# OSU-Nowlab/MPI4DL

Hardware: NVIDIA H100
Metric: images/sec (device-timed, max over ranks) AmoebaNet-D 8192^2 hot path (spatial-stage conv/pool fwd+bwd) (higher is better)
Workload: dtype bf16

## Files before the change

mpi4dl_b200/build.py:

```python
import os
import subprocess
import sys

HERE = os.path.dirname(os.path.abspath(__file__))
CSRC = os.path.join(HERE, "csrc")
LIB = os.path.join(HERE, "libspconv.so")
SOURCES = ["api.cu", "conv_direct.cu", "pool.cu", "halo.cu", "gemm_tc.cu", "conv_tap.cu", "wgrad_tap.cu", "bnrelu.cu",
           "halo_grad.cu", "gemm_tf32.cu", "conv_tap_tf32.cu", "conv_tap_s2_tf32.cu",
           "gemm_px.cu"]
NVCC_FLAGS = [
    "-O3", "-std=c++17", "-gencode", "arch=compute_90a,code=sm_90a", "-lineinfo",
    "-Xcompiler", "-fPIC", "--expt-relaxed-constexpr",
]


def _stale(target, deps):
    if not os.path.exists(target):
        return True
    t = os.path.getmtime(target)
    return any(os.path.getmtime(d) > t for d in deps)


def build_lib(force=False, verbose=False):
    nvcc = os.environ.get("NVCC", "/usr/local/cuda/bin/nvcc")
    hdrs = [os.path.join(CSRC, f) for f in os.listdir(CSRC) if f.endswith((".cuh", ".h"))]
    hdrs.append(os.path.join(HERE, "..", "include", "spconv.h"))
    objs = []
    procs = []
    for s in SOURCES:
        src = os.path.join(CSRC, s)
        obj = os.path.join(CSRC, s.replace(".cu", ".o"))
        objs.append(obj)
        if force or _stale(obj, [src] + hdrs):
            cmd = [nvcc] + NVCC_FLAGS + (["-Xptxas", "-v"] if verbose else []) + ["-c", src, "-o", obj]
            procs.append((s, subprocess.Popen(cmd, stdout=subprocess.PIPE, stderr=subprocess.STDOUT, text=True)))
    for s, p in procs:
        out, _ = p.communicate()
        if p.returncode != 0:
            sys.stderr.write(out)
            raise RuntimeError("nvcc failed on %s" % s)
        if verbose:
            sys.stderr.write(out)
    if force or procs or _stale(LIB, objs):
        cmd = [nvcc, "-shared", "-o", LIB] + objs + ["-gencode", "arch=compute_90a,code=sm_90a"]
        subprocess.check_call(cmd)
    return LIB


if __name__ == "__main__":
    print(build_lib(force="--force" in sys.argv, verbose="-v" in sys.argv))
```

mpi4dl_b200/csrc/gemm_tc.cu:

```cuda
#include <stdlib.h>

#include "common.cuh"
#include "tc_common.cuh"

namespace spc {

using namespace tc;

bool tap_v2_supported(int M, int Cin, int R, int S, int H, int W, int N, int stride);
int run_conv_tap_v2(const __nv_bfloat16* wp, int Mpad, int Cpad, const __nv_bfloat16* x, const __nv_bfloat16* bias,
                    __nv_bfloat16* y, int M, int Cin, int R, int S, int ph, int H, int W, int N, cudaStream_t st);

bool wgrad_tap_supported(int K, int C, int R, int S, int H, int W, int stride);
int run_wgrad_tap(const __nv_bfloat16* x, const __nv_bfloat16* dy, float* dw, int K, int C, int N, int H, int W, int R, int S,
                  cudaStream_t st);

int run_pw_px(int NT, const CUtensorMap& tw, const CUtensorMap& tx, const CUtensorMap& ty, int M, int Cin, int N, int P,
              int x5, int y5, const __nv_bfloat16* bias, int sms, cudaStream_t st);

namespace {

constexpr int TC_THREADS = 384;
constexpr int BK = 64;
constexpr int A_BLK_BYTES = 128 * BK * 2;
constexpr int B_BLK_BYTES = BK * 64 * 2;

typedef CUresult (*EncodeTiledFn)(CUtensorMap*, CUtensorMapDataType, cuuint32_t, void*, const cuuint64_t*,
                                  const cuuint64_t*, const cuuint32_t*, const cuuint32_t*, CUtensorMapInterleave,
                                  CUtensorMapSwizzle, CUtensorMapL2promotion, CUtensorMapFloatOOBfill);
EncodeTiledFn get_encode() {
  static EncodeTiledFn fn = nullptr;
  if (!fn) {
    void* p = nullptr;
    cudaDriverEntryPointQueryResult q;
    if (cudaGetDriverEntryPoint("cuTensorMapEncodeTiled", &p, cudaEnableDefault, &q) == cudaSuccess &&
        q == cudaDriverEntryPointSuccess)
      fn = reinterpret_cast<EncodeTiledFn>(p);
  }
  return fn;
}

int make_tmap_sw(CUtensorMap* m, const void* base, int rank, const uint64_t* dims, const uint64_t* strides_bytes,
                 const uint32_t* box, CUtensorMapSwizzle swz) {
  EncodeTiledFn enc = get_encode();
  if (!enc) {
    set_error("cuTensorMapEncodeTiled entry point not available");
    return SPC_ECUDA;
  }
  static thread_local bool ctx_bound = false;
  if (!ctx_bound) {
    if (cudaFree(nullptr) != cudaSuccess) {
      set_error("wgmma conv: no CUDA context on this thread");
      return SPC_ECUDA;
    }
    ctx_bound = true;
  }
  cuuint64_t gd[5], gs[5];
  cuuint32_t bx[5], es[5];
  for (int i = 0; i < rank; ++i) {
    gd[i] = dims[i];
    bx[i] = box[i];
    es[i] = 1;
    if (i > 0) gs[i - 1] = strides_bytes[i];
  }
  CUresult r = enc(m, CU_TENSOR_MAP_DATA_TYPE_BFLOAT16, (cuuint32_t)rank, const_cast<void*>(base), gd, gs, bx, es,
                   CU_TENSOR_MAP_INTERLEAVE_NONE, swz, CU_TENSOR_MAP_L2_PROMOTION_L2_256B,
                   CU_TENSOR_MAP_FLOAT_OOB_FILL_NONE);
  if (r != CUDA_SUCCESS) {
    set_error("cuTensorMapEncodeTiled failed (%d) rank=%d dims=[%llu,%llu,%llu] strides=[%llu,%llu]", (int)r, rank,
              (unsigned long long)dims[0], (unsigned long long)(rank > 1 ? dims[1] : 0),
              (unsigned long long)(rank > 2 ? dims[2] : 0), (unsigned long long)(rank > 1 ? strides_bytes[1] : 0),
              (unsigned long long)(rank > 2 ? strides_bytes[2] : 0));
    return SPC_ECUDA;
  }
  return SPC_OK;
}

int make_tmap(CUtensorMap* m, const void* base, int rank, const uint64_t* dims, const uint64_t* strides_bytes,
              const uint32_t* box) {
  return make_tmap_sw(m, base, rank, dims, strides_bytes, box, CU_TENSOR_MAP_SWIZZLE_128B);
}

__global__ void repack_weights_kernel(const __nv_bfloat16* __restrict__ w, __nv_bfloat16* __restrict__ wp, int M,
                                      int Cc, int Mpad, int Cpad, int taps, long long sm, long long sc, int flip) {
  const int total = taps * Mpad * Cpad;
  for (int i = blockIdx.x * blockDim.x + threadIdx.x; i < total; i += gridDim.x * blockDim.x) {
    const int c = i % Cpad;
    const int m = (i / Cpad) % Mpad;
    const int tap = i / (Cpad * Mpad);
    __nv_bfloat16 v = __float2bfloat16(0.f);
    if (m < M && c < Cc) v = w[(size_t)m * sm + (size_t)c * sc + (flip ? taps - 1 - tap : tap)];
    wp[i] = v;
  }
}
// ... 215 lines not shown
  }
  return sms;
}

constexpr int SMEM_LIMIT = 222 * 1024;
constexpr int SMEM_AUX = 1024  + 512 ;

template <int MB>
int launch_pw(const CUtensorMap& tw, const CUtensorMap& tx, const CUtensorMap& tx4, const CUtensorMap& ty, PwParams p,
              cudaStream_t st) {
  const int kchunks = (p.Cin + BK - 1) / BK;
  const int budget = SMEM_LIMIT - SMEM_AUX;
  const int wres_bytes = p.taps * kchunks * MB * A_BLK_BYTES;
  const int sms = sm_count();
  const int grid = p.num_tiles < sms ? p.num_tiles : sms;
  if (p.num_tiles < 16 * sms) p.tgroup = 1;
  p.wres = (wres_bytes <= 128 * 1024 && p.num_mg == 1) ? 1 : 0;
  const int stage_bytes = (p.wres ? 0 : MB * A_BLK_BYTES) + (BN / 64) * B_BLK_BYTES;
  const int rem = budget - (p.wres ? wres_bytes : 0);
  p.out_bufs = 2;
  p.stages = (rem - 2 * OUT_BUF_BYTES) / stage_bytes;
  if (p.stages < 3) { p.out_bufs = 1; p.stages = (rem - OUT_BUF_BYTES) / stage_bytes; }
  if (p.stages > MAX_STAGES) p.stages = MAX_STAGES;
  SPC_REQUIRE(p.stages >= 2, "wgmma conv: shared memory budget too small (MB=%d kchunks=%d)", MB, kchunks);
  const int smem = (p.wres ? wres_bytes : 0) + p.stages * stage_bytes + p.out_bufs * OUT_BUF_BYTES + SMEM_AUX;
  auto kern = pw_gemm_kernel<MB>;
  static bool attr_set = false;
  if (!attr_set) {
    SPC_CHECK_CUDA(cudaFuncSetAttribute(kern, cudaFuncAttributeMaxDynamicSharedMemorySize, SMEM_LIMIT));
    attr_set = true;
  }
  kern<<<grid, TC_THREADS, smem, st>>>(tw, tx, tx4, ty, p);
  count_launch();
  SPC_CHECK_CUDA(cudaGetLastError());
  return SPC_OK;
}

int make_act_tmap(CUtensorMap* m, const void* base, int P, int Cc, int N, int box_rows) {
  const uint64_t dims[3] = {(uint64_t)P, (uint64_t)Cc, (uint64_t)N};
  const uint64_t strides[3] = {0, (uint64_t)P * 2, (uint64_t)P * Cc * 2};
  const uint32_t box[3] = {64, (uint32_t)box_rows, 1};
  return make_tmap(m, base, 3, dims, strides, box);
}

int make_act_tmap5(CUtensorMap* m, const void* base, int P, int Cc, int N, int groups, int blocks) {
  const uint64_t dims[5] = {64, 8, (uint64_t)P / 64, (uint64_t)Cc / 8, (uint64_t)N};
  const uint64_t strides[5] = {0, (uint64_t)P * 2, 128, (uint64_t)P * 16, (uint64_t)P * Cc * 2};
  const uint32_t box[5] = {64, 8, (uint32_t)blocks, (uint32_t)groups, 1};
  return make_tmap(m, base, 5, dims, strides, box);
}

int launch_shift_copies(const void* x, void* xs, size_t planes, int H, int W, int S, int pw, int cs, cudaStream_t st);

struct TcConv {
  const __nv_bfloat16* w;
  long long sm, sc;
  int flip;
  int M, Cin;
  int R, S, ph, pw;
  int H, W, N;
  int stride;
  const __nv_bfloat16* prepacked;
  int px;
};

int px_tile_channels(int M) {
  const int nt = M <= 56 ? 56 : (M <= 104 ? 104 : 208);
  const int pad = round_up(M, nt);
  const int blocks = (M + 127) / 128;
  const int old_rows = (blocks >= 2 ? round_up(blocks, 2) : 1) * 128;
  return (pad < old_rows && 10 * M >= 9 * pad) ? nt : 0;
}

int run_conv_tc(const TcConv& c, const __nv_bfloat16* x, const __nv_bfloat16* bias, __nv_bfloat16* y, void* ws,
                size_t ws_bytes, cudaStream_t st) {
  const int taps = c.R * c.S;
  const int cs = c.stride;
  const int Ho = c.H / cs, Wo = c.W / cs;
  const int Pin = c.H * c.W, P = Ho * Wo;
  const int nt = (c.px && taps == 1) ? px_tile_channels(c.M) : 0;
  const bool px = nt && (long long)c.N * ((P + BN - 1) / BN) >= 2ll * sm_count();
  const int Mpad = round_up(c.M, px ? nt : 128), Cpad = round_up(c.Cin, BK);
  const bool v2 = taps > 1 && !env_get("SPC_TAP_V1") && tap_v2_supported(c.M, c.Cin, c.R, c.S, c.H, c.W, c.N, cs);
  const bool copies = (c.S > 1 || cs > 1) && taps > 1 && !v2;
  const uintptr_t ws0 = reinterpret_cast<uintptr_t>(ws);
  const uintptr_t wp_addr = (ws0 + 1023) & ~(uintptr_t)1023;
  const size_t wp_bytes = c.prepacked ? 0 : (size_t)taps * Mpad * Cpad * 2;
  const uintptr_t xs_addr = (wp_addr + wp_bytes + 1023) & ~(uintptr_t)1023;
  const size_t xs_bytes = copies ? (size_t)c.S * c.N * c.Cin * c.H * Wo * 2 : 0;
  const size_t need = (xs_addr - ws0) + xs_bytes;
  SPC_REQUIRE((ws && ws_bytes >= need) || need <= 1024, "wgmma conv: workspace too small (%zu < %zu)", ws_bytes, need);
  const __nv_bfloat16* wp = c.prepacked;
  if (!c.prepacked) {
    __nv_bfloat16* wpm = reinterpret_cast<__nv_bfloat16*>(wp_addr);
    const int total = taps * Mpad * Cpad;
    int blocks = (total + 255) / 256;
    if (blocks > 1184) blocks = 1184;
    repack_weights_kernel<<<blocks, 256, 0, st>>>(c.w, wpm, c.M, c.Cin, Mpad, Cpad, taps, c.sm, c.sc, c.flip);
    count_launch();
    SPC_CHECK_CUDA(cudaGetLastError());
    wp = wpm;
  }
  if (v2)
    return run_conv_tap_v2(wp, Mpad, Cpad, x, bias, y, c.M, c.Cin, c.R, c.S, c.ph, c.H, c.W, c.N, st);
  const __nv_bfloat16* xsrc = x;
  if (copies) {
    void* xs = reinterpret_cast<void*>(xs_addr);
    int rc0 = launch_shift_copies(x, xs, (size_t)c.N * c.Cin, c.H, c.W, c.S, c.pw, cs, st);
    if (rc0) return rc0;
    xsrc = reinterpret_cast<const __nv_bfloat16*>(xs);
  }
  CUtensorMap tw, tx, tx4, ty;
  const char* box5_env = env_get("SPC_PW_BOX5");
  const int box5 = box5_env ? atoi(box5_env) : ((size_t)P * 2 >= ((size_t)4 << 20) ? 3 : 0);
  const int x5 = (taps == 1 && cs == 1 && (box5 & 1) && P % 64 == 0 && c.Cin % 8 == 0) ? 1 : 0;
  const int y5 = (taps == 1 && (box5 & 2) && P % 64 == 0 && c.M % 8 == 0) ? 1 : 0;
  {
    const uint64_t dims[2] = {(uint64_t)Cpad, (uint64_t)taps * Mpad};
    const uint64_t strides[2] = {0, (uint64_t)Cpad * 2};
    const uint32_t box[2] = {BK, px ? (uint32_t)nt : 128u};
    int rc = make_tmap(&tw, wp, 2, dims, strides, box);
    if (rc) return rc;
  }
  int rc;
  if (px) {
    rc = x5 ? make_act_tmap5(&tx, x, Pin, c.Cin, c.N, BK / 8, BN / 64) : make_act_tmap(&tx, x, Pin, c.Cin, c.N, BK);
    if (rc) return rc;
    rc = y5 ? make_act_tmap5(&ty, y, P, c.M, c.N, nt / 8, 2) : make_act_tmap(&ty, y, P, c.M, c.N, nt);
    if (rc) return rc;
    return run_pw_px(nt, tw, tx, ty, c.M, c.Cin, c.N, P, x5, y5, bias, sm_count(), st);
  }
  if (taps > 1) {
    const uint64_t dims[4] = {(uint64_t)Wo, (uint64_t)c.H, (uint64_t)c.Cin, (uint64_t)c.N * (copies ? c.S : 1)};
    const uint64_t strides[4] = {0, (uint64_t)Wo * 2, (uint64_t)c.H * Wo * 2, (uint64_t)c.H * Wo * c.Cin * 2};
    const uint32_t box[4] = {64, 1, BK, 1};
    rc = make_tmap(&tx4, xsrc, 4, dims, strides, box);
    if (rc) return rc;
    tx = tx4;
  } else {
    rc = x5 ? make_act_tmap5(&tx, x, Pin, c.Cin, c.N, BK / 8, BN / 64) : make_act_tmap(&tx, x, Pin, c.Cin, c.N, BK);
    if (rc) return rc;
    tx4 = tx;
  }
  rc = y5 ? make_act_tmap5(&ty, y, P, c.M, c.N, 16, 2) : make_act_tmap(&ty, y, P, c.M, c.N, 128);
  if (rc) return rc;
  PwParams p{};
  p.x5 = x5; p.y5 = y5;
  p.bias = bias; p.M = c.M; p.Cin = c.Cin; p.P = P; p.N = c.N;
  p.taps = taps; p.S = c.S; p.ph = c.ph; p.pw = c.pw; p.W = Wo; p.Mpad = Mpad;
  p.shiftN = copies ? c.N : 0;
  p.rowmul = cs;
  {
    const char* e = env_get("SPC_TILE_GROUP");
    p.tgroup = e ? atoi(e) : 1;
    if (p.tgroup < 1) p.tgroup = 1;
  }
  const int MBtot = Mpad / 128;
  const int mb = MBtot >= 2 ? 2 : 1;
  p.num_mg = (MBtot + mb - 1) / mb;
  p.tiles_per_image = (P + BN - 1) / BN;
  p.num_tiles = p.tiles_per_image * c.N * p.num_mg;
  return mb == 2 ? launch_pw<2>(tw, tx, tx4, ty, p, st) : launch_pw<1>(tw, tx, tx4, ty, p, st);
}

int run_pw(const __nv_bfloat16* w, int ld, int transpose, int M, int Cin, const __nv_bfloat16* x,
           const __nv_bfloat16* bias, __nv_bfloat16* y, int N, int P, void* ws, size_t ws_bytes, cudaStream_t st,
           int px = 1) {
  TcConv c{};
  c.px = px;
  c.w = w;
  c.sm = transpose ? 1 : ld; c.sc = transpose ? ld : 1; c.flip = 0;
  c.M = M; c.Cin = Cin; c.R = 1; c.S = 1; c.ph = 0; c.pw = 0; c.H = 1; c.W = P; c.N = N; c.stride = 1;
  return run_conv_tc(c, x, bias, y, ws, ws_bytes, st);
}

constexpr int WG_ACC = 256;

struct WgParams {
  float* dw;
  int K, C, P, N;
  int nblk;
  int n_blocks;
  int MG;
  int mgroups;
  int splits;
// ... 492 lines not shown
    count_launch();
    SPC_CHECK_CUDA(cudaGetLastError());
    return SPC_OK;
  }
  if (aligned && cs == 2 && S == 3 && pw == 1 && W % 16 == 0) {
    const size_t tot = planes * H * (W / 16);
    size_t blocks = (tot + 255) / 256;
    if (blocks > 132 * 32) blocks = 132 * 32;
    shift_copies_s2k3_kernel<<<(int)blocks, 256, 0, st>>>((const __nv_bfloat16*)x, (__nv_bfloat16*)xs, planes, H, W);
    count_launch();
    SPC_CHECK_CUDA(cudaGetLastError());
    return SPC_OK;
  }
  const size_t total = planes * H * (W / cs / 8) * S;
  size_t blocks = (total + 255) / 256;
  if (blocks > 132 * 32) blocks = 132 * 32;
  shift_copies_kernel<<<(int)blocks, 256, 0, st>>>((const __nv_bfloat16*)x, (__nv_bfloat16*)xs, planes, H, W, S, pw, cs);
  count_launch();
  SPC_CHECK_CUDA(cudaGetLastError());
  return SPC_OK;
}

inline bool is_s2(const spc_conv_desc* d) { return d->stride_h == 2 && d->stride_w == 2; }
inline size_t align1k(size_t b) { return (b + 1023) & ~(size_t)1023; }

bool tap_shape_ok(const spc_conv_desc* d) {
  if (d->dtype != SPC_BF16) return false;
  if (d->R * d->S == 1 || d->R * d->S > 49) return false;
  if ((d->R & 1) == 0 || (d->S & 1) == 0) return false;
  const bool s1 = d->stride_h == 1 && d->stride_w == 1, s2 = d->stride_h == 2 && d->stride_w == 2;
  if (!s1 && !s2) return false;
  if (s2 && (d->H % 2 || d->W % 2)) return false;
  const int Wo = d->W / d->stride_w;
  if (Wo % 64 != 0) return false;
  return (long long)d->H * d->W < (1ll << 31);
}

bool pw_shape_ok(const spc_conv_desc* d) {
  if (d->dtype != SPC_BF16) return false;
  if (d->R != 1 || d->S != 1) return false;
  long long P = (long long)d->H * d->W;
  if (is_s2(d)) {
    if (d->H % 2 || d->W % 32) return false;
    P /= 4;
  } else if (d->stride_h != 1 || d->stride_w != 1) {
    return false;
  }
  if (P % 8 != 0 || P >= (1ll << 31)) return false;
  return true;
}

}

bool tc_supported(const spc_conv_desc* d, int op) {
  if (pw_shape_ok(d)) return true;
  if (tap_shape_ok(d)) {
    if (tc_workspace_bytes(d, op) > (24ull << 30)) return false;
    if (op == 1 && is_s2(d)) return d->R == 3 && d->S == 3 && 4 * d->C <= 2048;
    return true;
  }
  return false;
}

static size_t wbytes(const spc_conv_desc* d, int op) {
  const size_t taps = (size_t)d->R * d->S;
  if (op == 0) return align1k(taps * round_up(d->K, 128) * round_up(d->C, BK) * 2 + 1024);
  if (op == 1) return align1k(taps * round_up(d->C, 128) * round_up(d->K, BK) * 2 + 1024);
  return 0;
}
size_t tc_workspace_bytes(const spc_conv_desc* d, int op) {
  const size_t taps = (size_t)d->R * d->S;
  const int cs = d->stride_w;
  size_t b = wbytes(d, op) + 4096;
  if (taps == 1) {
    if (is_s2(d)) b += align1k((size_t)d->N * d->C * (d->H / 2) * (d->W / 2) * 2) + 1024;
    return b;
  }
  const size_t Ho = d->H / cs, Wo = d->W / cs;
  if (op == 1 && is_s2(d)) {
    b = align1k(4ull * round_up(4 * d->C, 128) * round_up(d->K, BK) * 2) + 4096;
    b += align1k(2ull * d->N * d->K * Ho * Wo * 2) + align1k(4ull * d->N * d->C * Ho * Wo * 2) + 4096;
    return b;
  }
  if (op != 2 && !env_get("SPC_TAP_V1") &&
      tap_v2_supported(op == 1 ? d->C : d->K, op == 1 ? d->K : d->C, d->R, d->S, d->H, d->W, d->N, cs))
    return b;
  if (op == 2 && !env_get("SPC_TAP_V1") && wgrad_tap_supported(d->K, d->C, d->R, d->S, d->H, d->W, cs))
    return b;
  if (d->S > 1 || cs > 1)
    b += align1k((size_t)d->S * d->N * (op == 1 ? d->K : d->C) * d->H * Wo * 2) + 2048;
  return b;
}

int tc_conv_fwd(const spc_conv_desc* d, const void* x, const void* w, const void* bias, void* y, void* ws,
                size_t ws_bytes, cudaStream_t st) {
  SPC_REQUIRE(ws && ws_bytes >= tc_workspace_bytes(d, 0), "wgmma conv: workspace too small");
  if (d->R * d->S > 1) {
    TcConv c{};
    c.w = reinterpret_cast<const __nv_bfloat16*>(w);
    c.sm = (long long)d->C * d->R * d->S; c.sc = (long long)d->R * d->S; c.flip = 0;
    c.M = d->K; c.Cin = d->C; c.R = d->R; c.S = d->S; c.ph = d->pad_h; c.pw = d->pad_w;
    c.H = d->H; c.W = d->W; c.N = d->N; c.stride = d->stride_h;
    return run_conv_tc(c, reinterpret_cast<const __nv_bfloat16*>(x), reinterpret_cast<const __nv_bfloat16*>(bias),
                       reinterpret_cast<__nv_bfloat16*>(y), ws, ws_bytes, st);
  }
  if (is_s2(d)) {
    void* xs = reinterpret_cast<void*>(align1k(reinterpret_cast<uintptr_t>(ws) + wbytes(d, 0)));
    int rc = launch_resample(false, x, xs, (size_t)d->N * d->C, d->H, d->W, st);
    if (rc) return rc;
    return run_pw(reinterpret_cast<const __nv_bfloat16*>(w), d->C, 0, d->K, d->C,
                  reinterpret_cast<const __nv_bfloat16*>(xs), reinterpret_cast<const __nv_bfloat16*>(bias),
                  reinterpret_cast<__nv_bfloat16*>(y), d->N, (d->H / 2) * (d->W / 2), ws, wbytes(d, 0), st);
  }
  return run_pw(reinterpret_cast<const __nv_bfloat16*>(w), d->C, 0, d->K, d->C,
                reinterpret_cast<const __nv_bfloat16*>(x), reinterpret_cast<const __nv_bfloat16*>(bias),
                reinterpret_cast<__nv_bfloat16*>(y), d->N, d->H * d->W, ws, ws_bytes, st);
}

int tc_conv_dgrad(const spc_conv_desc* d, const void* dy, const void* w, void* dx, void* ws, size_t ws_bytes,
                  cudaStream_t st) {
  SPC_REQUIRE(ws && ws_bytes >= tc_workspace_bytes(d, 1), "wgmma conv: workspace too small");
  if (d->R * d->S > 1 && is_s2(d)) {
    const int Ho = d->H / 2, Wo = d->W / 2;
    const int Mq = 4 * d->C, Mpad = round_up(Mq, 128), Kpad = round_up(d->K, BK);
    uintptr_t a = align1k(reinterpret_cast<uintptr_t>(ws));
    __nv_bfloat16* wq = reinterpret_cast<__nv_bfloat16*>(a);
    a = align1k(a + (size_t)4 * Mpad * Kpad * 2);
    __nv_bfloat16* tmp = reinterpret_cast<__nv_bfloat16*>(a);
    a = align1k(a + (size_t)4 * d->N * d->C * Ho * Wo * 2);
    {
      const int total = 4 * Mpad * Kpad;
      int blocks = (total + 255) / 256;
      if (blocks > 1184) blocks = 1184;
      repack_dgrad_s2_kernel<<<blocks, 256, 0, st>>>(reinterpret_cast<const __nv_bfloat16*>(w), wq, d->K, d->C, Mpad, Kpad);
      count_launch();
      SPC_CHECK_CUDA(cudaGetLastError());
    }
    TcConv c{};
    c.prepacked = wq;
    c.M = Mq; c.Cin = d->K; c.R = 2; c.S = 2; c.ph = 0; c.pw = 0; c.H = Ho; c.W = Wo; c.N = d->N; c.stride = 1;
    int rc = run_conv_tc(c, reinterpret_cast<const __nv_bfloat16*>(dy), nullptr, tmp, reinterpret_cast<void*>(a),
                         ws_bytes - (a - reinterpret_cast<uintptr_t>(ws)), st);
    if (rc) return rc;
    const size_t total = (size_t)d->N * d->C * 2 * Ho * (Wo / 8);
    size_t blocks = (total + 255) / 256;
    if (blocks > 132 * 32) blocks = 132 * 32;
    interleave_s2_kernel<<<(int)blocks, 256, 0, st>>>(tmp, reinterpret_cast<__nv_bfloat16*>(dx), d->N, d->C, Ho, Wo);
    count_launch();
    SPC_CHECK_CUDA(cudaGetLastError());
    return SPC_OK;
  }
  if (d->R * d->S > 1) {
    TcConv c{};
    c.w = reinterpret_cast<const __nv_bfloat16*>(w);
    c.sm = (long long)d->R * d->S; c.sc = (long long)d->C * d->R * d->S; c.flip = 1;
    c.M = d->C; c.Cin = d->K; c.R = d->R; c.S = d->S; c.ph = d->R - 1 - d->pad_h; c.pw = d->S - 1 - d->pad_w;
    c.H = d->H; c.W = d->W; c.N = d->N; c.stride = 1;
    return run_conv_tc(c, reinterpret_cast<const __nv_bfloat16*>(dy), nullptr, reinterpret_cast<__nv_bfloat16*>(dx), ws,
                       ws_bytes, st);
  }
  if (is_s2(d)) {
    void* gs = reinterpret_cast<void*>(align1k(reinterpret_cast<uintptr_t>(ws) + wbytes(d, 1)));
    int rc = run_pw(reinterpret_cast<const __nv_bfloat16*>(w), d->C, 1, d->C, d->K,
                    reinterpret_cast<const __nv_bfloat16*>(dy), nullptr, reinterpret_cast<__nv_bfloat16*>(gs), d->N,
                    (d->H / 2) * (d->W / 2), ws, wbytes(d, 1), st);
    if (rc) return rc;
    return launch_resample(true, gs, dx, (size_t)d->N * d->C, d->H, d->W, st);
  }
  return run_pw(reinterpret_cast<const __nv_bfloat16*>(w), d->C, 1, d->C, d->K,
                reinterpret_cast<const __nv_bfloat16*>(dy), nullptr, reinterpret_cast<__nv_bfloat16*>(dx), d->N,
                d->H * d->W, ws, ws_bytes, st);
}

int tc_conv_wgrad(const spc_conv_desc* d, const void* x, const void* dy, float* dw, int accumulate, void* ws,
                  size_t ws_bytes, cudaStream_t st) {
  (void)accumulate;
  const __nv_bfloat16* xb = reinterpret_cast<const __nv_bfloat16*>(x);
  const __nv_bfloat16* dyb = reinterpret_cast<const __nv_bfloat16*>(dy);
  if (d->R * d->S > 1) {
    const int cs = d->stride_h;
    if (!env_get("SPC_TAP_V1") && wgrad_tap_supported(d->K, d->C, d->R, d->S, d->H, d->W, cs))
      return run_wgrad_tap(xb, dyb, dw, d->K, d->C, d->N, d->H, d->W, d->R, d->S, st);
    const bool copies = d->S > 1 || cs > 1;
    if (copies) {
      SPC_REQUIRE(ws && ws_bytes >= tc_workspace_bytes(d, 2), "wgmma wgrad: workspace too small");
      void* xs = reinterpret_cast<void*>(align1k(reinterpret_cast<uintptr_t>(ws)));
      int rc = launch_shift_copies(x, xs, (size_t)d->N * d->C, d->H, d->W, d->S, d->pad_w, cs, st);
      if (rc) return rc;
      xb = reinterpret_cast<const __nv_bfloat16*>(xs);
    }
    return run_wgrad(xb, dyb, dw, d->K, d->C, d->N, d->H / cs, d->W / cs, d->H, d->R, d->S, d->pad_h, cs, copies, st);
  }
  if (is_s2(d)) {
    SPC_REQUIRE(ws && ws_bytes >= tc_workspace_bytes(d, 2), "wgmma wgrad: workspace too small");
    void* xs = reinterpret_cast<void*>(align1k(reinterpret_cast<uintptr_t>(ws)));
    int rc = launch_resample(false, x, xs, (size_t)d->N * d->C, d->H, d->W, st);
    if (rc) return rc;
    return run_wgrad(reinterpret_cast<const __nv_bfloat16*>(xs), dyb, dw, d->K, d->C, d->N, 1, (d->H / 2) * (d->W / 2), 1,
                     1, 1, 0, 1, false, st);
  }
  return run_wgrad(xb, dyb, dw, d->K, d->C, d->N, 1, d->H * d->W, 1, 1, 1, 0, 1, false, st);
}

size_t tc_pw_workspace_bytes(int M, int Cin) { return (size_t)round_up(M, 128) * round_up(Cin, BK) * 2 + 4096; }
int tc_pw_fwd(const void* w, int ld, int M, int Cin, const void* x, const void* bias, void* y, int P, void* ws, size_t ws_bytes,
              cudaStream_t st) {
  return run_pw(reinterpret_cast<const __nv_bfloat16*>(w), ld, 0, M, Cin, reinterpret_cast<const __nv_bfloat16*>(x),
                reinterpret_cast<const __nv_bfloat16*>(bias), reinterpret_cast<__nv_bfloat16*>(y), 1, P, ws, ws_bytes, st,
                0);
}
int tc_pw_wgrad(const void* x, const void* dy, float* dw, int K, int C, int P, cudaStream_t st) {
  return run_wgrad(reinterpret_cast<const __nv_bfloat16*>(x), reinterpret_cast<const __nv_bfloat16*>(dy), dw, K, C, 1, 1, P, 1, 1, 1,
                   0, 1, false, st);
}

int make_tmap_ex(CUtensorMap* m, const void* base, int rank, const uint64_t* dims, const uint64_t* strides_bytes,
                 const uint32_t* box, int swizzle128) {
  return make_tmap_sw(m, base, rank, dims, strides_bytes, box,
                      swizzle128 ? CU_TENSOR_MAP_SWIZZLE_128B : CU_TENSOR_MAP_SWIZZLE_NONE);
}
int tc_sm_count() { return sm_count(); }

}

extern "C" void spc_reload_env(void) { spc::g_env_n = 0; }
```

Before: 3.368.

## Add fused stride-2 3x3 tap conv and wgrad kernels with in-smem deinterleave

Result: faster. 3.463, median of 6 (+2.8%).

```diff
diff --git a/mpi4dl_b200/build.py b/mpi4dl_b200/build.py
--- a/mpi4dl_b200/build.py
+++ b/mpi4dl_b200/build.py
@@ -7,7 +7,7 @@
 LIB = os.path.join(HERE, "libspconv.so")
 SOURCES = ["api.cu", "conv_direct.cu", "pool.cu", "halo.cu", "gemm_tc.cu", "conv_tap.cu", "wgrad_tap.cu", "bnrelu.cu",
            "halo_grad.cu", "gemm_tf32.cu", "conv_tap_tf32.cu", "conv_tap_s2_tf32.cu",
-           "gemm_px.cu"]
+           "gemm_px.cu", "conv_tap_s2.cu"]
 NVCC_FLAGS = [
     "-O3", "-std=c++17", "-gencode", "arch=compute_90a,code=sm_90a", "-lineinfo",
     "-Xcompiler", "-fPIC", "--expt-relaxed-constexpr",
diff --git a/mpi4dl_b200/csrc/conv_tap_s2.cu b/mpi4dl_b200/csrc/conv_tap_s2.cu
--- /dev/null
+++ b/mpi4dl_b200/csrc/conv_tap_s2.cu
@@ -0,0 +1,597 @@
+#include "common.cuh"
+#include "tc_common.cuh"
+
+namespace spc {
+
+using namespace tc;
+
+int make_tmap_ex(CUtensorMap* m, const void* base, int rank, const uint64_t* dims, const uint64_t* strides_bytes,
+                 const uint32_t* box, int swizzle128);
+int tc_sm_count();
+
+namespace {
+
+constexpr int S2_THREADS = 640;
+constexpr int S2_NB = 2;
+constexpr int S2_ROWS = 2 * S2_NB + 1;
+constexpr int S2_TAPS = 9;
+constexpr int S2_RAW_PX = 136;
+constexpr int S2_RAW_ROW = S2_RAW_PX * 2;
+constexpr int S2_MAXRING = 8;
+constexpr int S2_STAGE_BYTES = 128 * 128;
+constexpr int S2_SHIFT_THREADS = 256;
+
+struct S2Params {
+  int M, Cin, H, W, N;
+  int Ho, Wo;
+  int Mpad;
+  int mrows, a_blk;
+  int kchunks, cbox;
+  int raw_blk, opblk;
+  int raw_buf;
+  int tiles_w, tiles_h, num_tiles;
+  int a_resident, ast, ops, rawb;
+  int group;
+  const __nv_bfloat16* bias;
+};
+
+struct Ring {
+  int s = 0, ph = 0;
+  __device__ __forceinline__ void next(int n) { if (++s == n) { s = 0; ph ^= 1; } }
+};
+
+struct S2Item {
+  uint4 a, b;
+  uint32_t prev;
+};
+__device__ __forceinline__ S2Item s2_load(const uint8_t* row, int q) {
+  S2Item it;
+  it.a = *reinterpret_cast<const uint4*>(row + 32 * q + 16);
+  it.b = *reinterpret_cast<const uint4*>(row + 32 * q + 32);
+  it.prev = *reinterpret_cast<const uint32_t*>(row + 32 * q + 12) >> 16;
+  return it;
+}
+template <int SI>
+__device__ __forceinline__ uint4 s2_tap(const S2Item& it) {
+  uint4 ev, od;
+  if (SI == 1) {
+    ev.x = __byte_perm(it.a.x, it.a.y, 0x5410); ev.y = __byte_perm(it.a.z, it.a.w, 0x5410);
+    ev.z = __byte_perm(it.b.x, it.b.y, 0x5410); ev.w = __byte_perm(it.b.z, it.b.w, 0x5410);
+    return ev;
+  }
+  od.x = __byte_perm(it.a.x, it.a.y, 0x7632); od.y = __byte_perm(it.a.z, it.a.w, 0x7632);
+  od.z = __byte_perm(it.b.x, it.b.y, 0x7632); od.w = __byte_perm(it.b.z, it.b.w, 0x7632);
+  if (SI == 2) return od;
+  uint4 sh;
+  sh.x = (od.x << 16) | it.prev;
+  sh.y = __funnelshift_r(od.x, od.y, 16);
+  sh.z = __funnelshift_r(od.y, od.z, 16);
+  sh.w = __funnelshift_r(od.z, od.w, 16);
+  return sh;
+}
+
+template <int SI>
+__device__ __forceinline__ void s2_store_tap(const S2Item (&it)[2 * S2_NB], int cv, int tid, uint8_t* op_base,
+                                             int opblk, int group, uint64_t* op_full, uint64_t* op_empty, Ring& ro,
+                                             int ops) {
+  const int q = tid & 7, c0 = tid >> 3;
+  const int tile_bytes = S2_NB * opblk;
+  if (!group || SI == 0) mbar_wait(&op_empty[ro.s], ro.ph ^ 1);
+  uint8_t* opb = op_base + ro.s * (group ? 3 : 1) * tile_bytes + (group ? SI * tile_bytes : 0);
+#pragma unroll
+  for (int i = 0; i < 2 * S2_NB; ++i) {
+    const int j = i >> 1, c = c0 + 32 * (i & 1);
+    if (c < cv) *reinterpret_cast<uint4*>(opb + j * opblk + c * 128 + ((q ^ (c & 7)) << 4)) = s2_tap<SI>(it[i]);
+  }
+  if (!group || SI == 2) {
+    fence_proxy_async();
+    mbar_arrive(&op_full[ro.s]);
+    ro.next(ops);
+  }
+}
+
+template <int KS>
+__global__ void __launch_bounds__(S2_THREADS, 1)
+conv_tap_s2_kernel(const __grid_constant__ CUtensorMap tmap_w, const __grid_constant__ CUtensorMap tmap_x,
+                   const __grid_constant__ CUtensorMap tmap_y, const S2Params p) {
+  constexpr int NPIX = S2_NB * 64;
+  extern __shared__ uint8_t smem_raw[];
+  uint8_t* smem = reinterpret_cast<uint8_t*>((reinterpret_cast<uintptr_t>(smem_raw) + 1023) & ~(uintptr_t)1023);
+  const int a_blocks = p.a_resident ? S2_TAPS * p.kchunks : p.ast;
+  const int raw_buf = p.raw_buf;
+  const int slot_bytes = (p.group ? 3 : 1) * S2_NB * p.opblk;
+  uint8_t* a_base = smem;
+  uint8_t* raw_base = a_base + a_blocks * p.a_blk;
+  uint8_t* op_base = raw_base + p.rawb * raw_buf;
+  uint8_t* stage_base = op_base + p.ops * slot_bytes;
+  uint8_t* bar_base = stage_base + S2_STAGE_BYTES;
+  uint64_t* raw_full = reinterpret_cast<uint64_t*>(bar_base);
+  uint64_t* raw_empty = raw_full + S2_MAXRING;
+  uint64_t* a_full = raw_empty + S2_MAXRING;
+  uint64_t* a_empty = a_full + S2_MAXRING;
+  uint64_t* op_full = a_empty + S2_MAXRING;
+  uint64_t* op_empty = op_full + S2_MAXRING;
+  uint64_t* a_res_full = op_empty + S2_MAXRING;
+
+  const int warp = threadIdx.x >> 5, lane = threadIdx.x & 31;
+
+  if (threadIdx.x == 0) {
+    for (int i = 0; i < S2_MAXRING; ++i) {
+      mbar_init(&raw_full[i], 1);
+      mbar_init(&raw_empty[i], S2_SHIFT_THREADS);
+      mbar_init(&a_full[i], 1); mbar_init(&a_empty[i], 2);
+      mbar_init(&op_full[i], S2_SHIFT_THREADS); mbar_init(&op_empty[i], 2);
+    }
+    mbar_init(a_res_full, 1);
+    fence_barrier_init();
+  }
+  __syncthreads();
+
+#define S2_TILE_DECODE(t)                                         \
+  const int tw_ = (t) % p.tiles_w;                                \
+  const int th_ = ((t) / p.tiles_w) % p.tiles_h;                  \
+  const int n_ = (t) / (p.tiles_w * p.tiles_h);                   \
+  const int w0 = tw_ * 64, h0 = th_ * S2_NB;
+
+  if (warp < 4) {
+    setmaxnreg_dec<24>();
+    if (warp == 0 && lane == 0) {
+      tma_prefetch_desc(&tmap_x);
+      tma_prefetch_desc(&tmap_w);
+      if (p.a_resident) {
+        mbar_arrive_expect_tx(a_res_full, S2_TAPS * p.kchunks * p.mrows * 128);
+        for (int tap = 0; tap < S2_TAPS; ++tap)
+          for (int kc = 0; kc < p.kchunks; ++kc)
+            tma_load_2d(a_base + (tap * p.kchunks + kc) * p.a_blk, &tmap_w, a_res_full, kc * 64, tap * p.Mpad);
+      }
+      Ring rb, ra;
+      int ct = blockIdx.x, ckc = 0;
+      if (ct < p.num_tiles) {
+        S2_TILE_DECODE(ct)
+        mbar_wait(&raw_empty[rb.s], rb.ph ^ 1);
+        mbar_arrive_expect_tx(&raw_full[rb.s], S2_ROWS * p.raw_blk);
+        for (int i = 0; i < S2_ROWS; ++i)
+          tma_load_4d(raw_base + rb.s * raw_buf + i * p.raw_blk, &tmap_x, &raw_full[rb.s], 2 * w0 - 8, 2 * h0 - 1 + i, 0, n_);
+        rb.next(p.rawb);
+      }
+      while (ct < p.num_tiles) {
+        int nt = ct, nkc = ckc + 1;
+        if (nkc == p.kchunks) { nkc = 0; nt = ct + gridDim.x; }
+        const bool has_next = nt < p.num_tiles;
+        S2_TILE_DECODE(has_next ? nt : ct)
+        uint8_t* dst = raw_base + rb.s * raw_buf;
+        bool armed = false;
+        int row = 0;
+        for (int tap = 0; tap < S2_TAPS; ++tap) {
+          if (!p.a_resident) {
+            mbar_wait(&a_empty[ra.s], ra.ph ^ 1);
+            mbar_arrive_expect_tx(&a_full[ra.s], p.mrows * 128);
+            tma_load_2d(a_base + ra.s * p.a_blk, &tmap_w, &a_full[ra.s], ckc * 64, tap * p.Mpad);
+            ra.next(p.ast);
+          }
+          if (has_next) {
+            if (!armed && mbar_test_wait(&raw_empty[rb.s], rb.ph ^ 1)) {
+              mbar_arrive_expect_tx(&raw_full[rb.s], S2_ROWS * p.raw_blk);
+              armed = true;
+            }
+            if (armed) {
+              const int quota = ((tap + 1) * S2_ROWS + S2_TAPS - 1) / S2_TAPS;
+              for (; row < quota; ++row)
+                tma_load_4d(dst + row * p.raw_blk, &tmap_x, &raw_full[rb.s], 2 * w0 - 8, 2 * h0 - 1 + row, nkc * 64, n_);
+            }
+          }
+        }
+        if (has_next) {
+          if (!armed) {
+            mbar_wait(&raw_empty[rb.s], rb.ph ^ 1);
+            mbar_arrive_expect_tx(&raw_full[rb.s], S2_ROWS * p.raw_blk);
+          }
+          for (; row < S2_ROWS; ++row)
+            tma_load_4d(dst + row * p.raw_blk, &tmap_x, &raw_full[rb.s], 2 * w0 - 8, 2 * h0 - 1 + row, nkc * 64, n_);
+          rb.next(p.rawb);
+        }
+        ct = nt; ckc = nkc;
+      }
+    }
+  } else if (warp >= 12) {
+    setmaxnreg_dec<80>();
+    const int tid = threadIdx.x - 12 * 32;
+    const int q = tid & 7, c0 = tid >> 3;
+    const int cv = p.cbox;
+    Ring rb, ro;
+    for (int t = blockIdx.x; t < p.num_tiles; t += gridDim.x) {
+      for (int kc = 0; kc < p.kchunks; ++kc) {
+        mbar_wait(&raw_full[rb.s], rb.ph);
+        const uint8_t* rawb = raw_base + rb.s * raw_buf;
+        for (int r = 0; r < 3; ++r) {
+          S2Item it[2 * S2_NB];
+#pragma unroll
+          for (int i = 0; i < 2 * S2_NB; ++i) {
+            const int j = i >> 1, c = c0 + 32 * (i & 1);
+            if (c < cv) it[i] = s2_load(rawb + (2 * j + r) * p.raw_blk + c * S2_RAW_ROW, q);
+          }
+          s2_store_tap<0>(it, cv, tid, op_base, p.opblk, p.group, op_full, op_empty, ro, p.ops);
+          s2_store_tap<1>(it, cv, tid, op_base, p.opblk, p.group, op_full, op_empty, ro, p.ops);
+          s2_store_tap<2>(it, cv, tid, op_base, p.opblk, p.group, op_full, op_empty, ro, p.ops);
+        }
+        mbar_arrive(&raw_empty[rb.s]);
+        rb.next(p.rawb);
+      }
+    }
+  } else {
+    setmaxnreg_inc<144>();
+    const int wg = (threadIdx.x >> 7) - 1;
+    const int w4 = (threadIdx.x >> 5) & 3;
+    const bool wg_lead = (threadIdx.x & 127) == 0;
+    const bool leader = threadIdx.x == 128;
+    float acc[NPIX / 2];
+    if (p.a_resident) mbar_wait(a_res_full, 0);
+    Ring ra, ro;
+    for (int t = blockIdx.x; t < p.num_tiles; t += gridDim.x) {
+      S2_TILE_DECODE(t)
+      int rel_op = -1, rel_a = -1;
+      for (int kc = 0; kc < p.kchunks; ++kc) {
+        for (int tap = 0; tap < S2_TAPS; ++tap) {
+          const int si = tap % 3;
+          if (!p.group || si == 0) mbar_wait(&op_full[ro.s], ro.ph);
+          const uint32_t sb = smem_u32(op_base + ro.s * slot_bytes + (p.group ? si * S2_NB * p.opblk : 0));
+          uint32_t sa;
+          if (p.a_resident) {
+            sa = smem_u32(a_base + (tap * p.kchunks + kc) * p.a_blk);
+          } else {
+            mbar_wait(&a_full[ra.s], ra.ph);
+            sa = smem_u32(a_base + ra.s * p.a_blk);
+          }
+          wgmma_fence();
+#pragma unroll
+          for (int ks = 0; ks < KS; ++ks) {
+            const uint64_t bdesc = gmma_desc(sb + ks * 2048, p.opblk, 1024);
+            const uint64_t adesc = gmma_desc(sa + wg * 8192 + ks * 32, 16, 1024);
+            Wgmma<NPIX, 1>::mma(acc, adesc, bdesc, (kc | tap | ks) ? 1u : 0u);
+          }
+          wgmma_commit();
+          wgmma_wait<1>();
+          if (wg_lead) {
+            if (rel_op >= 0) mbar_arrive(&op_empty[rel_op]);
+            if (rel_a >= 0) mbar_arrive(&a_empty[rel_a]);
+          }
+          rel_op = rel_a = -1;
+          if (!p.group || si == 2) { rel_op = ro.s; ro.next(p.ops); }
+          if (!p.a_resident) { rel_a = ra.s; ra.next(p.ast); }
+        }
+      }
+      wgmma_wait<0>();
+      reg_fence(acc);
+      if (wg_lead) {
+        if (rel_op >= 0) mbar_arrive(&op_empty[rel_op]);
+        if (rel_a >= 0) mbar_arrive(&a_empty[rel_a]);
+      }
+      const int r0 = 64 * wg + 16 * w4 + (lane >> 2);
+      const float b0 = (r0 < p.M && p.bias) ? __bfloat162float(p.bias[r0]) : 0.f;
+      const float b1 = (r0 + 8 < p.M && p.bias) ? __bfloat162float(p.bias[r0 + 8]) : 0.f;
+#pragma unroll
+      for (int j = 0; j < S2_NB; ++j) {
+        if (leader) tma_store_wait_read<0>();
+        named_bar_sync(1, 256);
+#pragma unroll
+        for (int qq = 0; qq < 8; ++qq) {
+#pragma unroll
+          for (int h = 0; h < 2; ++h) {
+            const int r = r0 + 8 * h;
+            const float bias = h ? b1 : b0;
+            const int i = 4 * (8 * j + qq) + 2 * h;
+            const uint32_t v = pack_bf16x2(acc[i] + bias, acc[i + 1] + bias);
+            *reinterpret_cast<uint32_t*>(stage_base + r * 128 + ((qq ^ (r & 7)) << 4) + (lane & 3) * 4) = v;
+          }
+        }
+        fence_proxy_async();
+        named_bar_sync(1, 256);
+        if (leader && h0 + j < p.Ho) {
+          tma_store_4d(&tmap_y, stage_base, w0, h0 + j, 0, n_);
+          tma_store_commit();
+        }
+      }
+    }
+    if (leader) tma_store_wait_read<0>();
+  }
+#undef S2_TILE_DECODE
+}
+
+constexpr int S2_SMEM_LIMIT = 222 * 1024;
+constexpr int S2_SMEM_AUX = 1024  + 1024 ;
+
+inline int round_up_i(int a, int b) { return (a + b - 1) / b * b; }
+
+bool plan_s2(int M, int Cin, S2Params* out, int* smem) {
+  S2Params p{};
+  p.M = M; p.Cin = Cin;
+  p.mrows = round_up_i(M, 8);
+  p.a_blk = round_up_i(p.mrows * 128, 1024);
+  p.kchunks = (Cin + 63) / 64;
+  p.cbox = Cin >= 64 ? 64 : round_up_i(Cin, 16);
+  p.raw_blk = p.cbox * S2_RAW_ROW;
+  p.opblk = p.cbox * 128;
+  p.raw_buf = round_up_i(S2_ROWS * p.raw_blk, 1024);
+  const int raw_buf = p.raw_buf;
+  const int budget = S2_SMEM_LIMIT - S2_SMEM_AUX - S2_STAGE_BYTES;
+  for (int resident = 1; resident >= 0; --resident) {
+    for (int group = 1; group >= 0; --group) {
+      const int slot = (group ? 3 : 1) * S2_NB * p.opblk;
+      int ast = resident ? 0 : 3;
+      const int a_bytes = resident ? S2_TAPS * p.kchunks * p.a_blk : ast * p.a_blk;
+      int rawb = 1, ops = 2;
+      int rem = budget - a_bytes - rawb * raw_buf - ops * slot;
+      if (rem < 0) continue;
+      if (rem >= raw_buf) { ++rawb; rem -= raw_buf; }
+      while (!resident && ast < S2_MAXRING && rem >= p.a_blk) { ++ast; rem -= p.a_blk; }
+      while (ops < 4 && rem >= slot) { ++ops; rem -= slot; }
+      p.a_resident = resident; p.ast = ast; p.ops = ops; p.rawb = rawb; p.group = group;
+      *out = p;
+      *smem = (resident ? a_bytes : ast * p.a_blk) + rawb * raw_buf + ops * slot + S2_STAGE_BYTES + S2_SMEM_AUX;
+      return true;
+    }
+  }
+  return false;
+}
+
+template <int KS>
+int launch_s2(const CUtensorMap& tw, const CUtensorMap& tx, const CUtensorMap& ty, const S2Params& p, int smem,
+              cudaStream_t st) {
+  auto kern = conv_tap_s2_kernel<KS>;
+  static bool attr_set = false;
+  if (!attr_set) {
+    SPC_CHECK_CUDA(cudaFuncSetAttribute(kern, cudaFuncAttributeMaxDynamicSharedMemorySize, S2_SMEM_LIMIT));
+    attr_set = true;
+  }
+  const int sms = tc_sm_count();
+  const int grid = p.num_tiles < sms ? p.num_tiles : sms;
+  kern<<<grid, S2_THREADS, smem, st>>>(tw, tx, ty, p);
+  count_launch();
+  SPC_CHECK_CUDA(cudaGetLastError());
+  return SPC_OK;
+}
+
+constexpr int W2_DY_ROW = 128 * 128;
+
+__global__ void __launch_bounds__(S2_THREADS, 1)
+wgrad_tap_s2_kernel(const __grid_constant__ CUtensorMap tmap_x, const __grid_constant__ CUtensorMap tmap_dy,
+                    float* __restrict__ dw, const S2Params p) {
+  extern __shared__ uint8_t smem_raw[];
+  uint8_t* smem = reinterpret_cast<uint8_t*>((reinterpret_cast<uintptr_t>(smem_raw) + 1023) & ~(uintptr_t)1023);
+  const int slot = p.raw_buf + S2_NB * W2_DY_ROW;
+  const int slot_bytes = 3 * S2_NB * p.opblk;
+  uint8_t* raw_base = smem;
+  uint8_t* op_base = raw_base + p.rawb * slot;
+  uint8_t* bar_base = op_base + p.ops * slot_bytes;
+  uint64_t* raw_full = reinterpret_cast<uint64_t*>(bar_base);
+  uint64_t* raw_empty = raw_full + S2_MAXRING;
+  uint64_t* op_full = raw_empty + S2_MAXRING;
+  uint64_t* op_empty = op_full + S2_MAXRING;
+
+  const int warp = threadIdx.x >> 5, lane = threadIdx.x & 31;
+  if (threadIdx.x == 0) {
+    for (int i = 0; i < S2_MAXRING; ++i) {
+      mbar_init(&raw_full[i], 1);
+      mbar_init(&raw_empty[i], S2_SHIFT_THREADS + 2);
+      mbar_init(&op_full[i], S2_SHIFT_THREADS); mbar_init(&op_empty[i], 2);
+    }
+    fence_barrier_init();
+  }
+  __syncthreads();
+
+#define W2_TILE_DECODE(t)                                         \
+  const int tw_ = (t) % p.tiles_w;                                \
+  const int th_ = ((t) / p.tiles_w) % p.tiles_h;                  \
+  const int n_ = (t) / (p.tiles_w * p.tiles_h);                   \
+  const int w0 = tw_ * 64, h0 = th_ * S2_NB;
+
+  if (warp < 4) {
+    setmaxnreg_dec<24>();
+    if (warp == 0 && lane == 0) {
+      tma_prefetch_desc(&tmap_x);
+      tma_prefetch_desc(&tmap_dy);
+      Ring rb;
+      for (int t = blockIdx.x; t < p.num_tiles; t += gridDim.x) {
+        W2_TILE_DECODE(t)
+        uint8_t* dst = raw_base + rb.s * slot;
+        mbar_wait(&raw_empty[rb.s], rb.ph ^ 1);
+        mbar_arrive_expect_tx(&raw_full[rb.s], S2_ROWS * p.raw_blk + S2_NB * W2_DY_ROW);
+        for (int i = 0; i < S2_ROWS; ++i)
+          tma_load_4d(dst + i * p.raw_blk, &tmap_x, &raw_full[rb.s], 2 * w0 - 8, 2 * h0 - 1 + i, 0, n_);
+        for (int j = 0; j < S2_NB; ++j)
+          tma_load_4d(dst + p.raw_buf + j * W2_DY_ROW, &tmap_dy, &raw_full[rb.s], w0, h0 + j, 0, n_);
+        rb.next(p.rawb);
+      }
+    }
+  } else if (warp >= 12) {
+    setmaxnreg_dec<80>();
+    const int tid = threadIdx.x - 12 * 32;
+    const int q = tid & 7, c0 = tid >> 3;
+    const int cv = p.cbox;
+    Ring rb, ro;
+    for (int t = blockIdx.x; t < p.num_tiles; t += gridDim.x) {
+      mbar_wait(&raw_full[rb.s], rb.ph);
+      const uint8_t* rawb = raw_base + rb.s * slot;
+      for (int r = 0; r < 3; ++r) {
+        S2Item it[2 * S2_NB];
+#pragma unroll
+        for (int i = 0; i < 2 * S2_NB; ++i) {
+          const int j = i >> 1, c = c0 + 32 * (i & 1);
+          if (c < cv) it[i] = s2_load(rawb + (2 * j + r) * p.raw_blk + c * S2_RAW_ROW, q);
+        }
+        s2_store_tap<0>(it, cv, tid, op_base, p.opblk, 1, op_full, op_empty, ro, p.ops);
+        s2_store_tap<1>(it, cv, tid, op_base, p.opblk, 1, op_full, op_empty, ro, p.ops);
+        s2_store_tap<2>(it, cv, tid, op_base, p.opblk, 1, op_full, op_empty, ro, p.ops);
+      }
+      mbar_arrive(&raw_empty[rb.s]);
+      rb.next(p.rawb);
+    }
+  } else {
+    setmaxnreg_inc<144>();
+    const int wg = (threadIdx.x >> 7) - 1;
+    const int w4 = (threadIdx.x >> 5) & 3;
+    const bool wg_lead = (threadIdx.x & 127) == 0;
+    float acc[S2_TAPS][8];
+#pragma unroll
+    for (int t = 0; t < S2_TAPS; ++t)
+#pragma unroll
+      for (int i = 0; i < 8; ++i) acc[t][i] = 0.f;
+    Ring rb, ro;
+    for (int t = blockIdx.x; t < p.num_tiles; t += gridDim.x) {
+      mbar_wait(&raw_full[rb.s], rb.ph);
+      const uint32_t sdy = smem_u32(raw_base + rb.s * slot + p.raw_buf);
+#pragma unroll
+      for (int r = 0; r < 3; ++r) {
+        mbar_wait(&op_full[ro.s], ro.ph);
+        const uint32_t sb = smem_u32(op_base + ro.s * slot_bytes);
+        wgmma_fence();
+#pragma unroll
+        for (int s = 0; s < 3; ++s)
+#pragma unroll
+          for (int j = 0; j < S2_NB; ++j)
+#pragma unroll
+            for (int ks = 0; ks < 4; ++ks) {
+              const uint64_t adesc = gmma_desc(sdy + j * W2_DY_ROW + wg * 8192 + ks * 32, 16, 1024);
+              const uint64_t bdesc = gmma_desc(sb + (s * S2_NB + j) * p.opblk + ks * 32, 16, 1024);
+              Wgmma<16, 0>::mma(acc[3 * r + s], adesc, bdesc, 1u);
+            }
+        wgmma_commit();
+        wgmma_wait<0>();
+        if (wg_lead) mbar_arrive(&op_empty[ro.s]);
+        ro.next(p.ops);
+      }
+      if (wg_lead) mbar_arrive(&raw_empty[rb.s]);
+      rb.next(p.rawb);
+    }
+    const int m0 = 64 * wg + 16 * w4 + (lane >> 2);
+#pragma unroll
+    for (int tap = 0; tap < S2_TAPS; ++tap)
+#pragma unroll
+      for (int i = 0; i < 8; ++i) {
+        const int m = m0 + 8 * ((i >> 1) & 1);
+        const int c = 8 * (i >> 2) + 2 * (lane & 3) + (i & 1);
+        if (m < p.M && c < p.Cin) atomicAdd(&dw[((size_t)m * p.Cin + c) * S2_TAPS + tap], acc[tap][i]);
+      }
+  }
+#undef W2_TILE_DECODE
+}
+
+bool plan_w2(int M, int Cin, S2Params* out, int* smem) {
+  if (M > 128 || Cin > 16) return false;
+  S2Params p{};
+  p.M = M; p.Cin = Cin;
+  p.kchunks = 1;
+  p.cbox = 16;
+  p.raw_blk = p.cbox * S2_RAW_ROW;
+  p.opblk = p.cbox * 128;
+  p.raw_buf = round_up_i(S2_ROWS * p.raw_blk, 1024);
+  p.rawb = 2;
+  p.ops = 4;
+  p.group = 1;
+  *out = p;
+  *smem = p.rawb * (p.raw_buf + S2_NB * W2_DY_ROW) + p.ops * 3 * S2_NB * p.opblk + S2_SMEM_AUX;
+  return *smem <= S2_SMEM_LIMIT;
+}
+
+}
+
+bool tap_s2_supported(int M, int Cin, int R, int S, int ph, int pw, int H, int W, int N) {
+  if (R != 3 || S != 3 || ph != 1 || pw != 1 || M > 128 || (H & 1) || (W & 1)) return false;
+  const int Ho = H / 2, Wo = W / 2;
+  if (Wo % 64 != 0) return false;
+  const long long tiles = (long long)N * ((Ho + S2_NB - 1) / S2_NB) * (Wo / 64);
+  if (tiles < 2ll * tc_sm_count()) return false;
+  S2Params p;
+  int smem;
+  return plan_s2(M, Cin, &p, &smem);
+}
+
+int run_conv_tap_s2(const __nv_bfloat16* wp, int Mpad, int Cpad, const __nv_bfloat16* x, const __nv_bfloat16* bias,
+                    __nv_bfloat16* y, int M, int Cin, int H, int W, int N, cudaStream_t st) {
+  S2Params p;
+  int smem;
+  SPC_REQUIRE(plan_s2(M, Cin, &p, &smem), "stride-2 tap conv: no shared-memory plan for M=%d Cin=%d", M, Cin);
+  p.H = H; p.W = W; p.N = N; p.Ho = H / 2; p.Wo = W / 2;
+  p.Mpad = Mpad; p.bias = bias;
+  p.tiles_w = p.Wo / 64;
+  p.tiles_h = (p.Ho + S2_NB - 1) / S2_NB;
+  p.num_tiles = p.tiles_w * p.tiles_h * N;
+  CUtensorMap tw, tx, ty;
+  {
+    const uint64_t dims[2] = {(uint64_t)Cpad, (uint64_t)S2_TAPS * Mpad};
+    const uint64_t strides[2] = {0, (uint64_t)Cpad * 2};
+    const uint32_t box[2] = {64, (uint32_t)p.mrows};
+    int rc = make_tmap_ex(&tw, wp, 2, dims, strides, box, 1);
+    if (rc) return rc;
+  }
+  {
+    const uint64_t dims[4] = {(uint64_t)W, (uint64_t)H, (uint64_t)Cin, (uint64_t)N};
+    const uint64_t strides[4] = {0, (uint64_t)W * 2, (uint64_t)H * W * 2, (uint64_t)H * W * Cin * 2};
+    const uint32_t box[4] = {S2_RAW_PX, 1, (uint32_t)p.cbox, 1};
+    int rc = make_tmap_ex(&tx, x, 4, dims, strides, box, 0);
+    if (rc) return rc;
+  }
+  {
+    const uint64_t dims[4] = {(uint64_t)p.Wo, (uint64_t)p.Ho, (uint64_t)M, (uint64_t)N};
+    const uint64_t strides[4] = {0, (uint64_t)p.Wo * 2, (uint64_t)p.Ho * p.Wo * 2, (uint64_t)p.Ho * p.Wo * M * 2};
+    const uint32_t box[4] = {64, 1, 128, 1};
+    int rc = make_tmap_ex(&ty, y, 4, dims, strides, box, 1);
+    if (rc) return rc;
+  }
+  switch (p.cbox / 16) {
+    case 1: return launch_s2<1>(tw, tx, ty, p, smem, st);
+    case 2: return launch_s2<2>(tw, tx, ty, p, smem, st);
+    case 3: return launch_s2<3>(tw, tx, ty, p, smem, st);
+    default: return launch_s2<4>(tw, tx, ty, p, smem, st);
+  }
+}
+
+bool wgrad_tap_s2_supported(int M, int Cin, int R, int S, int ph, int pw, int H, int W, int N) {
+  if (R != 3 || S != 3 || ph != 1 || pw != 1 || (H & 1) || (W & 1)) return false;
+  const int Ho = H / 2, Wo = W / 2;
+  if (Wo % 64 != 0) return false;
+  const long long tiles = (long long)N * ((Ho + S2_NB - 1) / S2_NB) * (Wo / 64);
+  if (tiles < 2ll * tc_sm_count()) return false;
+  S2Params p;
+  int smem;
+  return plan_w2(M, Cin, &p, &smem);
+}
+
+int run_wgrad_tap_s2(const __nv_bfloat16* x, const __nv_bfloat16* dy, float* dw, int M, int Cin, int H, int W, int N,
+                     cudaStream_t st) {
+  S2Params p;
+  int smem;
+  SPC_REQUIRE(plan_w2(M, Cin, &p, &smem), "stride-2 tap wgrad: no plan for M=%d Cin=%d", M, Cin);
+  p.H = H; p.W = W; p.N = N; p.Ho = H / 2; p.Wo = W / 2;
+  p.tiles_w = p.Wo / 64;
+  p.tiles_h = (p.Ho + S2_NB - 1) / S2_NB;
+  p.num_tiles = p.tiles_w * p.tiles_h * N;
+  CUtensorMap tx, tdy;
+  {
+    const uint64_t dims[4] = {(uint64_t)W, (uint64_t)H, (uint64_t)Cin, (uint64_t)N};
+    const uint64_t strides[4] = {0, (uint64_t)W * 2, (uint64_t)H * W * 2, (uint64_t)H * W * Cin * 2};
+    const uint32_t box[4] = {S2_RAW_PX, 1, (uint32_t)p.cbox, 1};
+    int rc = make_tmap_ex(&tx, x, 4, dims, strides, box, 0);
+    if (rc) return rc;
+  }
+  {
+    const uint64_t dims[4] = {(uint64_t)p.Wo, (uint64_t)p.Ho, (uint64_t)M, (uint64_t)N};
+    const uint64_t strides[4] = {0, (uint64_t)p.Wo * 2, (uint64_t)p.Ho * p.Wo * 2, (uint64_t)p.Ho * p.Wo * M * 2};
+    const uint32_t box[4] = {64, 1, 128, 1};
+    int rc = make_tmap_ex(&tdy, dy, 4, dims, strides, box, 1);
+    if (rc) return rc;
+  }
+  static bool attr_set = false;
+  if (!attr_set) {
+    SPC_CHECK_CUDA(cudaFuncSetAttribute(wgrad_tap_s2_kernel, cudaFuncAttributeMaxDynamicSharedMemorySize, S2_SMEM_LIMIT));
+    attr_set = true;
+  }
+  const int sms = tc_sm_count();
+  const int grid = p.num_tiles < sms ? p.num_tiles : sms;
+  wgrad_tap_s2_kernel<<<grid, S2_THREADS, smem, st>>>(tx, tdy, dw, p);
+  count_launch();
+  SPC_CHECK_CUDA(cudaGetLastError());
+  return SPC_OK;
+}
+
+}
diff --git a/mpi4dl_b200/csrc/gemm_tc.cu b/mpi4dl_b200/csrc/gemm_tc.cu
--- a/mpi4dl_b200/csrc/gemm_tc.cu
+++ b/mpi4dl_b200/csrc/gemm_tc.cu
@@ -10,6 +10,13 @@
 bool tap_v2_supported(int M, int Cin, int R, int S, int H, int W, int N, int stride);
 int run_conv_tap_v2(const __nv_bfloat16* wp, int Mpad, int Cpad, const __nv_bfloat16* x, const __nv_bfloat16* bias,
                     __nv_bfloat16* y, int M, int Cin, int R, int S, int ph, int H, int W, int N, cudaStream_t st);
+
+bool tap_s2_supported(int M, int Cin, int R, int S, int ph, int pw, int H, int W, int N);
+int run_conv_tap_s2(const __nv_bfloat16* wp, int Mpad, int Cpad, const __nv_bfloat16* x, const __nv_bfloat16* bias,
+                    __nv_bfloat16* y, int M, int Cin, int H, int W, int N, cudaStream_t st);
+bool wgrad_tap_s2_supported(int M, int Cin, int R, int S, int ph, int pw, int H, int W, int N);
+int run_wgrad_tap_s2(const __nv_bfloat16* x, const __nv_bfloat16* dy, float* dw, int M, int Cin, int H, int W, int N,
+                     cudaStream_t st);
 
 bool wgrad_tap_supported(int K, int C, int R, int S, int H, int W, int stride);
 int run_wgrad_tap(const __nv_bfloat16* x, const __nv_bfloat16* dy, float* dw, int K, int C, int N, int H, int W, int R, int S,
@@ -391,7 +398,8 @@
   const bool px = nt && (long long)c.N * ((P + BN - 1) / BN) >= 2ll * sm_count();
   const int Mpad = round_up(c.M, px ? nt : 128), Cpad = round_up(c.Cin, BK);
   const bool v2 = taps > 1 && !env_get("SPC_TAP_V1") && tap_v2_supported(c.M, c.Cin, c.R, c.S, c.H, c.W, c.N, cs);
-  const bool copies = (c.S > 1 || cs > 1) && taps > 1 && !v2;
+  const bool s2 = cs == 2 && !c.prepacked && tap_s2_supported(c.M, c.Cin, c.R, c.S, c.ph, c.pw, c.H, c.W, c.N);
+  const bool copies = (c.S > 1 || cs > 1) && taps > 1 && !v2 && !s2;
   const uintptr_t ws0 = reinterpret_cast<uintptr_t>(ws);
   const uintptr_t wp_addr = (ws0 + 1023) & ~(uintptr_t)1023;
   const size_t wp_bytes = c.prepacked ? 0 : (size_t)taps * Mpad * Cpad * 2;
@@ -410,6 +418,7 @@
     SPC_CHECK_CUDA(cudaGetLastError());
     wp = wpm;
   }
+  if (s2) return run_conv_tap_s2(wp, Mpad, Cpad, x, bias, y, c.M, c.Cin, c.H, c.W, c.N, st);
   if (v2)
     return run_conv_tap_v2(wp, Mpad, Cpad, x, bias, y, c.M, c.Cin, c.R, c.S, c.ph, c.H, c.W, c.N, st);
   const __nv_bfloat16* xsrc = x;
@@ -1068,6 +1077,10 @@
     b += align1k(2ull * d->N * d->K * Ho * Wo * 2) + align1k(4ull * d->N * d->C * Ho * Wo * 2) + 4096;
     return b;
   }
+  if (op == 0 && is_s2(d) && tap_s2_supported(d->K, d->C, d->R, d->S, d->pad_h, d->pad_w, d->H, d->W, d->N))
+    return b;
+  if (op == 2 && is_s2(d) && wgrad_tap_s2_supported(d->K, d->C, d->R, d->S, d->pad_h, d->pad_w, d->H, d->W, d->N))
+    return b;
   if (op != 2 && !env_get("SPC_TAP_V1") &&
       tap_v2_supported(op == 1 ? d->C : d->K, op == 1 ? d->K : d->C, d->R, d->S, d->H, d->W, d->N, cs))
     return b;
@@ -1165,6 +1178,8 @@
   const __nv_bfloat16* dyb = reinterpret_cast<const __nv_bfloat16*>(dy);
   if (d->R * d->S > 1) {
     const int cs = d->stride_h;
+    if (is_s2(d) && wgrad_tap_s2_supported(d->K, d->C, d->R, d->S, d->pad_h, d->pad_w, d->H, d->W, d->N))
+      return run_wgrad_tap_s2(xb, dyb, dw, d->K, d->C, d->H, d->W, d->N, st);
     if (!env_get("SPC_TAP_V1") && wgrad_tap_supported(d->K, d->C, d->R, d->S, d->H, d->W, cs))
       return run_wgrad_tap(xb, dyb, dw, d->K, d->C, d->N, d->H, d->W, d->R, d->S, st);
     const bool copies = d->S > 1 || cs > 1;
```
